# indrajeetadityaroy9/rabitq-ann-search

Hardware: AMD Instinct MI355X
Metric: qps (search_batch_device, layer-0 hot path end to end) + fastscan_dist_per_s (higher is better)
Workload: dtype u32 popcount / f32; 1 GPU; SIFT1M-class synthetic (int-valued, clustered; SURVEY 8d C2): 1000000x128 f32 (D=128), 4-bit RaBitQ FastScan + exact-L2 rerank, R=32, k=10, 10000 queries per GPU resident in HBM; n_index=1000000, dim=128, bits=4, k=10, nq_per_gpu=10000, index_builder=cphnsw_mi355x (this repo), batch_sets=2, parallelism=query-sharded x1, index replicated

## Files before the change

include/cphnsw_mi355x.h:

```cpp
#ifndef CPHNSW_MI355X_H
#define CPHNSW_MI355X_H

#include <stddef.h>
#include <stdint.h>

#ifdef __cplusplus
extern "C" {
#endif

typedef struct cph_index cph_index;

typedef enum {
    CPH_OK = 0,
    CPH_INVALID_ARGUMENT = 1,
    CPH_RUNTIME_ERROR = 2,
    CPH_OUT_OF_MEMORY = 3,
    CPH_NOT_IMPLEMENTED = 4
} cph_status;

const char* cph_last_error(void);

int cph_version(void);

int cph_create(uint64_t dim, uint64_t bits, int device, cph_index** out);
// ... 293 lines not shown
                                        int64_t* d_ids, float* d_dist, void* stream);
int cph_parts_search_batch_filters_device(cph_parts* m, const float* d_queries, uint64_t n, uint64_t k,
                                          const cph_parts_filter* const* filters, uint32_t n_filters, const int32_t* filter_of,
                                          int exact, int64_t* d_ids, float* d_dist, void* stream);
int cph_parts_search(cph_parts* m, const float* query, uint64_t k, int64_t* ids, float* dist, uint64_t* count);
int cph_parts_set_exact_threshold(cph_parts* m, uint64_t max_allowed);
int cph_parts_filter_create_rows(cph_parts* m, const uint32_t* words, uint64_t n_bits, cph_parts_filter** out);
int cph_parts_filter_destroy(cph_parts_filter* f);
int cph_parts_last_search_stats(cph_parts* m, uint64_t out[13]);
int cph_parts_last_query_expansions(cph_parts* m, uint32_t* out, uint64_t n);
int cph_parts_remove(cph_parts* m, const int64_t* ids, uint64_t cnt, uint64_t* newly);
int cph_parts_live_count(cph_parts* m, uint64_t* n);
int cph_parts_get_removed(cph_parts* m, uint32_t* words);
int cph_parts_compact(cph_parts* m, int64_t* old_to_new);
int cph_multi_set_labels(cph_multi* m, const int32_t* labels, uint64_t n, int space);
int cph_parts_set_labels(cph_parts* m, const int32_t* labels, uint64_t n);
int cph_parts_filters_from_labels(cph_parts* m, const int32_t* lo, const int32_t* hi, uint32_t cnt, cph_parts_filter** out);
int cph_parts_filter_count(const cph_parts_filter* f, uint64_t* count);
int cph_multi_set_column(cph_multi* m, uint32_t slot, const int32_t* values, uint64_t n, int space);
int cph_parts_set_column(cph_parts* m, uint32_t slot, const int32_t* values, uint64_t n);
int cph_parts_filters_from_column(cph_parts* m, uint32_t slot, const int32_t* lo, const int32_t* hi, uint32_t cnt, cph_parts_filter** out);
int cph_parts_filters_combine(int op, const cph_parts_filter* const* a, uint32_t m, const cph_parts_filter* const* b, uint32_t n_b,
                              cph_parts_filter** out);
int cph_parts_num_parts(cph_parts* m, uint32_t* n);
int cph_parts_part(cph_parts* m, uint32_t i, cph_index** out);
int cph_parts_bounds(cph_parts* m, uint64_t* out);
int cph_merge_rows_hook(int device, const int64_t* ids, const float* dist, uint32_t P, uint64_t n, uint64_t k, const int64_t* lo,
                        int64_t* out_ids, float* out_dist);

int cph_encode_query(cph_index* h, const float* query, uint8_t* lut, float* coeffs);

int cph_entry_point(cph_index* h, const float* query, uint32_t* entry);

int cph_fastscan_block(cph_index* h, const uint8_t* lut, const float* qparams,
                       uint32_t vertex, float dist_qp_sq, float worst, int nn_full,
                       uint32_t* sums, uint32_t* msb, float* est, float* lower,
                       float* lower_stage1);

int cph_exact_l2(cph_index* h, const float* query, const uint32_t* ids, uint64_t n,
                 float* out);

typedef struct cph_stream cph_stream;
int cph_fastscan_stream_create(int device, uint32_t D, uint32_t bits, uint64_t n_blocks,
                               uint64_t seed, cph_stream** out, uint64_t* block_bytes);
int cph_fastscan_stream_run(cph_stream* s, int reps, double* avg_ms, double* checksum);
int cph_fastscan_stream_export(cph_stream* s, uint64_t first, uint64_t count,
                               uint8_t* ref_blocks, uint8_t* lut, float* qparams,
                               float* dist_qp_sq);
int cph_fastscan_stream_eval(cph_stream* s, uint64_t first, uint64_t count, float* est,
                             float* lower);
int cph_fastscan_stream_destroy(cph_stream* s);

int cph_host_rewrite_index(const char* path_in, const char* path_out);
int cph_host_repack_block(uint32_t D, uint32_t bits, const uint8_t* ref_block, uint8_t* dev_block,
                          uint64_t* dev_bytes, uint8_t* ref_roundtrip);
int cph_host_relayout_block(uint32_t D, uint32_t bits, const uint8_t* dev_block, uint8_t* resident_block,
                            uint8_t* dev_roundtrip);
int cph_export_blocks(cph_index* h, uint64_t first, uint64_t count, int resident, uint8_t* out);
int cph_host_encode_query(uint64_t dim, const float* query, uint8_t* lut, float* coeffs, uint32_t* masks);
int cph_host_rows_filter(const uint32_t* words_in, const uint32_t* rows, uint64_t n, uint32_t* words_out);

int cph_host_live_filter(const uint32_t* words_f, const uint32_t* words_removed, uint64_t n, uint32_t* words_out,
                         uint64_t* count_out);

int cph_host_filter_ids(const uint32_t* words, uint64_t n_bits, uint32_t* out_ids, uint64_t* out_count);
int cph_host_exact_plan(uint64_t candidates, uint64_t n_queries, uint64_t k, int num_cus, uint64_t scratch_bytes, uint64_t* out);
// ... 60 lines not shown
```

rabitq-ann-search_amd/cphnsw_mi355x/_lib.py:

```python
import ctypes as C
import importlib.util
import os
import sys

from . import build as _build

OK, INVALID_ARGUMENT, RUNTIME_ERROR, OUT_OF_MEMORY, NOT_IMPLEMENTED = range(5)
IDS_INTERNAL, IDS_INPUT = 0, 1
METRIC_L2, METRIC_COSINE = 0, 1
METRIC_IP = 2

SYMBOLS = {
    "cph_last_error": (C.c_char_p, []),
    "cph_version": (C.c_int, []),
    "cph_create": (C.c_int, [C.c_uint64, C.c_uint64, C.c_int, C.POINTER(C.c_void_p)]),
    "cph_destroy": (C.c_int, [C.c_void_p]),
    "cph_load": (C.c_int, [C.c_void_p, C.c_char_p]),
    "cph_save": (C.c_int, [C.c_void_p, C.c_char_p]),
    "cph_save_native": (C.c_int, [C.c_void_p, C.c_char_p]),
    "cph_load_native": (C.c_int, [C.c_void_p, C.c_char_p]),
    "cph_size": (C.c_int, [C.c_void_p, C.POINTER(C.c_uint64)]),
    "cph_dim": (C.c_int, [C.c_void_p, C.POINTER(C.c_uint64)]),
    "cph_is_finalized": (C.c_int, [C.c_void_p, C.POINTER(C.c_int)]),
    "cph_build": (C.c_int, [C.c_void_p, C.c_void_p, C.c_uint64]),
# ... 201 lines not shown
    "cph_parts_size": (C.c_int, [C.c_void_p, C.POINTER(C.c_uint64)]),
    "cph_parts_is_finalized": (C.c_int, [C.c_void_p, C.POINTER(C.c_int)]),
    "cph_parts_save_native": (C.c_int, [C.c_void_p, C.c_char_p]),
    "cph_parts_load_native": (C.c_int, [C.c_void_p, C.c_char_p]),
    "cph_parts_search_batch": (C.c_int, [C.c_void_p, C.c_void_p, C.c_uint64, C.c_uint64, C.c_void_p, C.c_void_p]),
    "cph_parts_search_batch_filtered": (C.c_int, [C.c_void_p, C.c_void_p, C.c_uint64, C.c_uint64, C.c_void_p, C.c_void_p,
                                                  C.c_void_p]),
    "cph_parts_search_batch_exact": (C.c_int, [C.c_void_p, C.c_void_p, C.c_uint64, C.c_uint64, C.c_void_p, C.c_void_p,
                                               C.c_void_p]),
    "cph_parts_search_batch_filters": (C.c_int, [C.c_void_p, C.c_void_p, C.c_uint64, C.c_uint64, C.c_void_p, C.c_uint32,
                                                 C.c_void_p, C.c_int, C.c_void_p, C.c_void_p]),
    "cph_parts_search_batch_device": (C.c_int, [C.c_void_p, C.c_void_p, C.c_uint64, C.c_uint64, C.c_void_p, C.c_void_p,
                                                C.c_void_p]),
    "cph_parts_search_batch_device_filtered": (C.c_int, [C.c_void_p, C.c_void_p, C.c_uint64, C.c_uint64, C.c_void_p,
                                                         C.c_void_p, C.c_void_p, C.c_void_p]),
    "cph_parts_search_batch_exact_device": (C.c_int, [C.c_void_p, C.c_void_p, C.c_uint64, C.c_uint64, C.c_void_p,
                                                      C.c_void_p, C.c_void_p, C.c_void_p]),
    "cph_parts_search_batch_filters_device": (C.c_int, [C.c_void_p, C.c_void_p, C.c_uint64, C.c_uint64, C.c_void_p, C.c_uint32,
                                                        C.c_void_p, C.c_int, C.c_void_p, C.c_void_p, C.c_void_p]),
    "cph_parts_search": (C.c_int, [C.c_void_p, C.c_void_p, C.c_uint64, C.c_void_p, C.c_void_p, C.POINTER(C.c_uint64)]),
    "cph_parts_set_exact_threshold": (C.c_int, [C.c_void_p, C.c_uint64]),
    "cph_parts_filter_create_rows": (C.c_int, [C.c_void_p, C.c_void_p, C.c_uint64, C.POINTER(C.c_void_p)]),
    "cph_parts_filter_destroy": (C.c_int, [C.c_void_p]),
    "cph_parts_last_search_stats": (C.c_int, [C.c_void_p, C.POINTER(C.c_uint64)]),
    "cph_parts_last_query_expansions": (C.c_int, [C.c_void_p, C.c_void_p, C.c_uint64]),
    "cph_parts_num_parts": (C.c_int, [C.c_void_p, C.POINTER(C.c_uint32)]),
    "cph_parts_part": (C.c_int, [C.c_void_p, C.c_uint32, C.POINTER(C.c_void_p)]),
    "cph_parts_bounds": (C.c_int, [C.c_void_p, C.c_void_p]),
    "cph_merge_rows_hook": (C.c_int, [C.c_int, C.c_void_p, C.c_void_p, C.c_uint32, C.c_uint64, C.c_uint64, C.c_void_p,
                                      C.c_void_p, C.c_void_p]),
    "cph_host_part_bounds": (C.c_int, [C.c_uint64, C.c_uint32, C.c_void_p]),
    "cph_encode_query": (C.c_int, [C.c_void_p, C.c_void_p, C.c_void_p, C.c_void_p]),
    "cph_entry_point": (C.c_int, [C.c_void_p, C.c_void_p, C.POINTER(C.c_uint32)]),
    "cph_fastscan_block": (C.c_int, [C.c_void_p, C.c_void_p, C.c_void_p, C.c_uint32, C.c_float, C.c_float,
                                     C.c_int, C.c_void_p, C.c_void_p, C.c_void_p, C.c_void_p, C.c_void_p]),
    "cph_exact_l2": (C.c_int, [C.c_void_p, C.c_void_p, C.c_void_p, C.c_uint64, C.c_void_p]),
    "cph_host_rewrite_index": (C.c_int, [C.c_char_p, C.c_char_p]),
    "cph_host_repack_block": (C.c_int, [C.c_uint32, C.c_uint32, C.c_void_p, C.c_void_p, C.POINTER(C.c_uint64), C.c_void_p]),
    "cph_host_relayout_block": (C.c_int, [C.c_uint32, C.c_uint32, C.c_void_p, C.c_void_p, C.c_void_p]),
    "cph_export_blocks": (C.c_int, [C.c_void_p, C.c_uint64, C.c_uint64, C.c_int, C.c_void_p]),
    "cph_host_encode_query": (C.c_int, [C.c_uint64, C.c_void_p, C.c_void_p, C.c_void_p, C.c_void_p]),
    "cph_host_rows_filter": (C.c_int, [C.c_void_p, C.c_void_p, C.c_uint64, C.c_void_p]),
    "cph_fastscan_stream_create": (C.c_int, [C.c_int, C.c_uint32, C.c_uint32, C.c_uint64, C.c_uint64,
                                             C.POINTER(C.c_void_p), C.POINTER(C.c_uint64)]),
    "cph_fastscan_stream_run": (C.c_int, [C.c_void_p, C.c_int, C.POINTER(C.c_double), C.POINTER(C.c_double)]),
    "cph_fastscan_stream_export": (C.c_int, [C.c_void_p, C.c_uint64, C.c_uint64, C.c_void_p, C.c_void_p,
                                             C.c_void_p, C.POINTER(C.c_float)]),
    "cph_fastscan_stream_eval": (C.c_int, [C.c_void_p, C.c_uint64, C.c_uint64, C.c_void_p, C.c_void_p]),
    "cph_fastscan_stream_destroy": (C.c_int, [C.c_void_p]),
    "cph_set_metric": (C.c_int, [C.c_void_p, C.c_int]),
    "cph_get_metric": (C.c_int, [C.c_void_p, C.POINTER(C.c_int)]),
    "cph_multi_set_metric": (C.c_int, [C.c_void_p, C.c_int]),
    "cph_parts_set_metric": (C.c_int, [C.c_void_p, C.c_int]),
    "cph_metric_stats": (C.c_int, [C.c_void_p, C.POINTER(C.c_uint64)]),
    "cph_normalize_rows_hook": (C.c_int, [C.c_int, C.c_void_p, C.c_uint64, C.c_uint64, C.c_void_p, C.POINTER(C.c_uint64),
                                          C.POINTER(C.c_uint64)]),
    "cph_host_normalize_rows": (C.c_int, [C.c_void_p, C.c_uint64, C.c_uint64, C.c_void_p, C.POINTER(C.c_uint64),
                                          C.POINTER(C.c_uint64)]),
    "cph_set_metric_ip": (C.c_int, [C.c_void_p]),
    "cph_multi_set_metric_ip": (C.c_int, [C.c_void_p]),
    "cph_set_ip_bound": (C.c_int, [C.c_void_p, C.c_float]),
    "cph_get_ip_bound": (C.c_int, [C.c_void_p, C.POINTER(C.c_float)]),
    "cph_multi_set_ip_bound": (C.c_int, [C.c_void_p, C.c_float]),
    "cph_multi_get_ip_bound": (C.c_int, [C.c_void_p, C.POINTER(C.c_float)]),
    "cph_ip_augment_hook": (C.c_int, [C.c_int, C.c_void_p, C.c_uint64, C.c_uint64, C.c_int, C.c_float, C.c_void_p, C.c_void_p,
                                      C.POINTER(C.c_float), C.POINTER(C.c_uint64)]),
# ... 83 lines not shown
```

rabitq-ann-search_amd/cphnsw_mi355x/build.py:

```python
import os
import shutil
import subprocess

PKG_DIR = os.path.dirname(os.path.abspath(__file__))
CSRC = os.path.join(os.path.dirname(PKG_DIR), "csrc")
LIB_PATH = os.path.join(PKG_DIR, "libcphnsw_mi355x.so")
SOURCES = ["cphnsw_mi355x.hip"]
HEADERS = ["cph_core.h", "builder.h", "builder_host.h", "host_parallel.h", "search_coalescer.h", "multi_device.h", "partitioned.h", "device_merge.h", "builder_pipeline.h", "device_knn.h", "device_knn_sym.h", "device_build.h", "device_buf.h", "native_file.h", "device_encode.h", "device_fastscan.h", "device_search.h", "device_search_expansion.inc", "device_stream.h", "device_heap_test.h", "device_relayout.h", "device_rows.h", "device_tombstone.h", "device_labels.h", "device_filter_ops.h", "device_exact.h", "device_range.h", "device_tail.h", "host_tail.h", "device_group.h", "host_group.h", "device_diverse.h", "host_diverse.h", "device_maxsim.h", "host_maxsim.h", "device_maxsim_rescore.h", "host_maxsim_rescore.h", "device_fused.h", "host_fused.h", "device_normalize.h", "host_normalize.h", "device_ip.h", "host_ip.h", "device_rescore.h", "host_rescore.h", "host_index.h"]
FLAGS = ["-O3", "-std=c++17", "--offload-arch=gfx950", "-fPIC", "-shared", "-ffp-contract=off",
         "-Wall", "-Wno-unused-function"]


def _hipcc():
    for c in (os.environ.get("HIPCC"), shutil.which("hipcc"), "/opt/rocm/bin/hipcc"):
        if c and os.path.exists(c):
            return c
    raise RuntimeError("hipcc not found (need ROCm to build the gfx950 library)")


def needs_build():
    if not os.path.exists(LIB_PATH):
        return True
    t = os.path.getmtime(LIB_PATH)
    deps = [os.path.join(CSRC, f) for f in SOURCES + HEADERS]
    deps.append(os.path.join(os.path.dirname(os.path.dirname(PKG_DIR)), "include", "cphnsw_mi355x.h"))
    return any(os.path.getmtime(d) > t for d in deps if os.path.exists(d))


def build_library(force=False, verbose=False):
    if not force and not needs_build():
        return LIB_PATH
    cmd = [_hipcc()] + FLAGS + [os.path.join(CSRC, s) for s in SOURCES] + ["-o", LIB_PATH, "-lpthread"]
    if verbose:
        print(" ".join(cmd))
    subprocess.check_call(cmd)
    return LIB_PATH


if __name__ == "__main__":
    print(build_library(force=True, verbose=True))
```

rabitq-ann-search_amd/csrc/cphnsw_mi355x.hip:

```cpp
#include <hip/hip_runtime.h>

#include <algorithm>
#include <atomic>
#include <cfloat>
#include <chrono>
#include <condition_variable>
#include <deque>
#include <functional>
#include <memory>
#include <mutex>
#include <new>
#include <shared_mutex>
#include <string>
#include <thread>
#include <vector>

#include "../../include/cphnsw_mi355x.h"
#include "cph_core.h"
#include "device_buf.h"
#include "device_encode.h"
#include "device_fastscan.h"
#include "device_search.h"
#include "device_stream.h"
#include "device_heap_test.h"
#include "device_relayout.h"
#include "device_rows.h"
#include "device_tombstone.h"
#include "device_labels.h"
#include "device_filter_ops.h"
#include "device_exact.h"
#include "device_range.h"
#include "device_tail.h"
#include "device_diverse.h"
#include "device_group.h"
#include "device_maxsim.h"
#include "device_maxsim_rescore.h"
#include "device_fused.h"
#include "device_rescore.h"
#include "device_normalize.h"
#include "device_ip.h"
#include "host_index.h"
#include "host_parallel.h"
#include "search_coalescer.h"
#include "multi_device.h"
#include "partitioned.h"
#include "device_merge.h"
#include "native_file.h"
#include "builder_pipeline.h"

using namespace cph;

namespace {

thread_local std::string g_err;

int fail(int code, const std::string& msg) {
    g_err = msg;
    return code;
}

struct InvalidArg : std::invalid_argument {
    using std::invalid_argument::invalid_argument;
};
struct NotImplemented : std::runtime_error {
    using std::runtime_error::runtime_error;
};

template <class F>
int guarded(F&& f) {
    try {
        f();
        return CPH_OK;
    } catch (const std::invalid_argument& e) {
// ... 157 lines not shown
    float ip_bound = 0.0f, ip_m2 = 0.0f;
    std::vector<float> pending;
    uint64_t pending_n = 0;
    HostIndex host;
    DevLayout L{};
    SearchConsts sc{};
    uint32_t flags = 0;
    int num_cus = 256;
    bool waves_from_env = false;
    uint32_t waves_per_cu = 4 * CPH_SEARCH_WAVES_PER_SIMD;
    DevBuf<uint8_t> d_blocks;
    DevBuf<float> d_raw, d_norm;
    DevBuf<uint32_t> d_rows;
    bool has_rows = false;
    bool ids_input = false;
    DevBuf<int32_t> d_labels, d_label_bounds;
    DevBuf<unsigned long long> d_label_counts;
    bool has_labels = false;
    std::unique_ptr<KeyRows> label_rows;
    DevBuf<int32_t> d_columns[kMaxColumns];
    bool has_column[kMaxColumns] = {};
    size_t exact_scratch_bytes = (size_t)1 << 30;
    uint64_t exact_threshold = 0;
    DevBuf<uint32_t> d_removed;
    DevBuf<unsigned long long> d_rm_count;
    uint64_t rm_epoch = 0;
    std::shared_ptr<cph_filter> live;
    std::atomic<bool> tombstones{false};
    uint64_t tail = 0;
    std::vector<float> tail_vecs;
    std::atomic<bool> has_tail{false};
    DevBuf<float> d_signs;
    DevBuf<uint32_t> d_upper;
    DevBuf<uint32_t> d_row_of;
    DevBuf<uint32_t> d_nbr_info;
    UpperLayerDev layers[kMaxUpperLayers];
    int32_t dev_max_level = 0;
    float norm_factor = 0.0f, inv_sqrt_d = 0.0f;
    NativeMapping native_map;
    const uint8_t* own_view = nullptr;
    std::vector<uint8_t> own_store;
    BatchSet sets[kMaxBatchSets + kLeaderSlots];
    int n_sets = 2;
    int last_set = kMaxBatchSets - 1;
    int last_search = -1;
    bool last_range = false;
    uint64_t range_exact = 0;
    std::vector<std::unique_ptr<RangeScratch>> range_scratch;
    GroupScratch group_scratch[kMaxBatchSets];
    int last_group = kMaxBatchSets - 1;
    struct PassTimer {
        hipEvent_t ev0 = nullptr, ev1 = nullptr;
        bool on = false, timed = false;
    } pass_timer[kPassKinds];
    uint64_t index_epoch = 0;
    hipStream_t own_stream = nullptr;
    bool order_queries = true;
    uint32_t want_slots = 0;
    uint64_t want_cap = 0;
    uint64_t auto_cap = 0;
    bool pf_off = false;
    bool pf_dense = false;
    std::mutex mu;
    SearchCoalescer coal;
    struct LeaderSlot {
        hipStream_t stream = nullptr;
        uint8_t* pin = nullptr;
        uint8_t* pin_dev = nullptr;
// ... 234 lines not shown
    if (n != 0) {
        DevBuf<uint32_t> d_flag(1);
        HIP_CHECK(hipMemset(d_flag.p, 0, 4));
        hipLaunchKernelGGL(scan_counts_kernel, dim3((uint32_t)((n + 255) / 256)), dim3(256), 0, nullptr, h->d_blocks.p, (uint64_t)n,
                           h->L.stride, h->L.count_off, d_flag.p);
        HIP_CHECK(hipGetLastError());
        uint32_t f = 0;
        HIP_CHECK(hipMemcpy(&f, d_flag.p, 4, hipMemcpyDeviceToHost));
        h->flags |= f & 2u;
    }
    h->d_signs.alloc(3 * hi.D);
    HIP_CHECK(hipMemcpy(h->d_signs.p, hi.rot.signs.data(), 3 * hi.D * 4, hipMemcpyHostToDevice));
    const float d = static_cast<float>(hi.D);
    h->norm_factor = 1.0f / (d * std::sqrt(d));
    h->inv_sqrt_d = 1.0f / std::sqrt(d);
    const int nl = std::min<int>({(int)hi.upper.size(), (int)hi.max_level, kMaxUpperLayers});
    h->dev_max_level = hi.max_level > 0 ? nl : 0;
    std::vector<uint32_t> flat;
    std::vector<size_t> off_nodes(nl), off_offs(nl), off_nbrs(nl);
    for (int l = 0; l < nl; ++l) {
        const auto& layer = hi.upper[l];
        off_nodes[l] = flat.size();
        for (const auto& e : layer) flat.push_back(e.node);
        off_offs[l] = flat.size();
        uint32_t acc = 0;
        for (const auto& e : layer) { flat.push_back(acc); acc += (uint32_t)e.nbrs.size(); }
        flat.push_back(acc);
        off_nbrs[l] = flat.size();
        for (const auto& e : layer) flat.insert(flat.end(), e.nbrs.begin(), e.nbrs.end());
    }
    h->d_upper.alloc(flat.size() + 1);
    if (!flat.empty())
        HIP_CHECK(hipMemcpy(h->d_upper.p, flat.data(), flat.size() * 4, hipMemcpyHostToDevice));
    for (int l = 0; l < kMaxUpperLayers; ++l) h->layers[l] = UpperLayerDev{nullptr, nullptr, nullptr, nullptr, nullptr, 0};
    int mapped = 0;
    size_t mapped_edges = 0;
    for (int l = 0; l < nl; ++l) {
        if (hi.upper[l].size() <= 16) continue;
        ++mapped;
        for (const auto& e : hi.upper[l]) mapped_edges += e.nbrs.size();
    }
    h->d_row_of.alloc((size_t)mapped * n + 1);
    h->d_nbr_info.alloc(mapped_edges + 1);
    std::vector<uint32_t> row_of, nbr_info;
    size_t info_off = 0;
    for (int l = 0, m = 0; l < nl; ++l) {
        const uint32_t* dmap = nullptr;
        const uint32_t* dinfo = nullptr;
        if (hi.upper[l].size() > 16) {
            row_of.assign(n, kInvalidNode);
            uint64_t first = 0;
            bool fits = true;
            for (size_t r = 0; r < hi.upper[l].size(); ++r) {
                const uint64_t deg = hi.upper[l][r].nbrs.size();
                if (first >= (1u << 26) || deg > 62) { fits = false; break; }
                row_of[hi.upper[l][r].node] = (uint32_t)first | ((uint32_t)deg << 26);
                first += deg;
            }
            if (!fits) { h->layers[l] = UpperLayerDev{h->d_upper.p + off_nodes[l], h->d_upper.p + off_offs[l], h->d_upper.p + off_nbrs[l], nullptr, nullptr, (uint32_t)hi.upper[l].size()}; ++m; continue; }
            HIP_CHECK(hipMemcpy(h->d_row_of.p + (size_t)m * n, row_of.data(), n * 4, hipMemcpyHostToDevice));
            dmap = h->d_row_of.p + (size_t)m * n;
            ++m;
            nbr_info.clear();
            for (const auto& e : hi.upper[l])
                for (const uint32_t nb : e.nbrs) nbr_info.push_back(nb < n ? row_of[nb] : kInvalidNode);
            if (info_off + nbr_info.size() > mapped_edges) throw std::runtime_error("upper layers: edge count changed during upload");
            if (!nbr_info.empty())
                HIP_CHECK(hipMemcpy(h->d_nbr_info.p + info_off, nbr_info.data(), nbr_info.size() * 4, hipMemcpyHostToDevice));
            dinfo = h->d_nbr_info.p + info_off;
            info_off += nbr_info.size();
        }
        h->layers[l] = UpperLayerDev{h->d_upper.p + off_nodes[l], h->d_upper.p + off_offs[l],
                                     h->d_upper.p + off_nbrs[l], dmap, dinfo, (uint32_t)hi.upper[l].size()};
    }
    for (auto& s : h->sets) release_scratch(s);
    reset_adaptation(h);
}

void materialize_search_data(cph_index* h) {
    HostIndex& hi = h->host;
    if (!hi.search_data.empty() || hi.n == 0) return;
    h->use_device();
    quiesce(h);
    const size_t n = hi.n, stride = h->L.stride, own_stride = hi.RL.nb_off;
    hi.search_data.assign(n * hi.RL.vertex_bytes, 0);
    const size_t chunk = std::max<size_t>(1, std::min<size_t>(n, (512u << 20) / stride));
    std::vector<uint8_t> stage(chunk * stride);
    for (size_t base = 0; base < n; base += chunk) {
        const size_t c = std::min(chunk, n - base);
        download_blocks(h->d_blocks.p + base * stride, c, h->L, stage.data());
        parallel_for(c, 256, [&](size_t lo, size_t hi_) {
            for (size_t v = lo; v < hi_; ++v) {
                uint8_t* dst = &hi.search_data[(base + v) * hi.RL.vertex_bytes];
                if (h->own_view) std::memcpy(dst, h->own_view + (base + v) * own_stride, own_stride);
                repack_dev_to_ref(&stage[v * stride], h->L, hi.RL, dst + hi.RL.nb_off);
            }
        });
    }
}

void init_set(BatchSet& s) {
    if (s.ev0) return;
    HIP_CHECK(hipEventCreate(&s.ev0));
    HIP_CHECK(hipEventCreate(&s.ev1));
    HIP_CHECK(hipEventCreateWithFlags(&s.ev_done, hipEventDisableTiming));
    HIP_CHECK(hipHostMalloc(reinterpret_cast<void**>(&s.pin_stats), kStatWords * 8, hipHostMallocDefault));
    std::memset(s.pin_stats, 0, kStatWords * 8);
// ... 2650 lines not shown
        const uint32_t D = h->D, PW = h->L.PW;
        std::vector<uint32_t> masks(PW * 4);
        QueryHeader hd;
        HIP_CHECK(hipMemcpy(masks.data(), s.d_qmasks.p, PW * 16, hipMemcpyDeviceToHost));
        HIP_CHECK(hipMemcpy(&hd, s.d_qhdr.p, sizeof(hd), hipMemcpyDeviceToHost));
        std::vector<uint8_t> qu(D);
        for (uint32_t d = 0; d < D; ++d) {
            uint8_t u = 0;
            for (int j = 0; j < 4; ++j) u |= (uint8_t)(((masks[(d / 32) * 4 + j] >> (d % 32)) & 1u) << j);
            qu[d] = u;
        }
        qu_to_lut(qu.data(), D, lut);
        coeffs[0] = hd.A; coeffs[1] = hd.B; coeffs[2] = hd.C;
    });
}

int cph_entry_point(cph_index* h, const float* query, uint32_t* entry) {
    return guarded([&] {
        std::lock_guard<std::mutex> lk(h->mu);
        require_finalized(h);
        h->use_device();
        hipStream_t st = own_stream(h);
        BatchSet& s = next_set(h, st);
        stage_queries(h, s, upload_queries(h, s, query, 1, st, true), 1, st);
        HIP_CHECK(hipEventRecord(s.ev_done, st));
        s.used = true;
        HIP_CHECK(hipStreamSynchronize(st));
        QueryHeader hd;
        HIP_CHECK(hipMemcpy(&hd, s.d_qhdr.p, sizeof(hd), hipMemcpyDeviceToHost));
        *entry = hd.entry;
    });
}

int cph_fastscan_block(cph_index* h, const uint8_t* lut, const float* qparams, uint32_t vertex,
                       float dist_qp_sq, float worst, int nn_full, uint32_t* sums, uint32_t* msb,
                       float* est, float* lower, float* lower_stage1) {
    return guarded([&] {
        std::lock_guard<std::mutex> lk(h->mu);
        require_finalized(h);
        if (vertex >= h->host.n) throw InvalidArg("vertex out of range");
        h->use_device();
        const uint32_t D = h->D, PW = h->L.PW;
        std::vector<uint8_t> qu(D);
        lut_to_qu(lut, D, qu.data());
        std::vector<uint32_t> masks(PW * 4);
        qu_to_masks(qu.data(), D, masks.data());
        DevBuf<uint4> d_mask;
        DevBuf<uint32_t> d_u;
        DevBuf<float> d_f;
        d_mask.alloc(PW);
        d_u.alloc(64);
        d_f.alloc(96);
        HIP_CHECK(hipMemcpy(d_mask.p, masks.data(), PW * 16, hipMemcpyHostToDevice));
        BlockHookArgs a{};
        a.blk = h->d_blocks.p + (size_t)vertex * h->L.stride;
        a.L = h->L;
        a.qmask = d_mask.p;
        a.qp = QP{qparams[0], qparams[1], qparams[2], qparams[3], qparams[4], qparams[5], qparams[6]};
        a.dqp = dist_qp_sq;
        a.worst = worst;
        a.nn_full = nn_full;
        a.sums = d_u.p; a.msb = d_u.p + 32;
        a.est = d_f.p; a.lower = d_f.p + 32; a.lower1 = d_f.p + 64;
        CPH_LAUNCH(block_hook_kernel, h->bits, D, dim3(1), dim3(64), (size_t)PW * 16, nullptr, a);
        HIP_CHECK(hipDeviceSynchronize());
        uint32_t hu[64];
// ... 373 lines not shown
    HIP_CHECK(hipDeviceSynchronize());
    begin_device_swap(dst);
    dst->host = host_scalars(src->host);
    dst->host.removed = src->host.removed;
    dst->host.n_removed = src->host.n_removed;
    drop_host_state(dst);
    dst->L = src->L;
    dst->sc = src->sc;
    dst->flags = src->flags;
    dst->dev_max_level = src->dev_max_level;
    dst->norm_factor = src->norm_factor;
    dst->inv_sqrt_d = src->inv_sqrt_d;
    dst->ip_m2 = src->ip_m2;
    hipStream_t st = own_stream(dst);
    auto copy = [&](auto& d, const auto& s) {
        d.alloc(s.n);
        if (s.n) HIP_CHECK(hipMemcpyPeerAsync(d.p, dst->device, s.p, src->device, s.n * sizeof(*s.p), st));
    };
    copy(dst->d_blocks, src->d_blocks);
    copy(dst->d_raw, src->d_raw);
    copy(dst->d_norm, src->d_norm);
    if (src->has_rows) copy(dst->d_rows, src->d_rows);
    else dst->d_rows.release();
    dst->has_rows = src->has_rows;
    dst->ids_input = dst->ids_input && dst->has_rows;
    for (int slot = kLabelSlot; slot < (int)kMaxColumns; ++slot) {
        const ColumnRef from = column_of(src, slot), to = column_of(dst, slot);
        if (from.has) copy(to.dev, from.dev);
        else to.dev.release();
        to.has = from.has;
    }
    copy(dst->d_signs, src->d_signs);
    copy(dst->d_upper, src->d_upper);
    copy(dst->d_row_of, src->d_row_of);
    copy(dst->d_nbr_info, src->d_nbr_info);
    HIP_CHECK(hipStreamSynchronize(st));
    sync_removed(dst);
    auto rebase = [](const uint32_t* p, const DevBuf<uint32_t>& from, const DevBuf<uint32_t>& to) -> const uint32_t* {
        return p ? to.p + (p - from.p) : nullptr;
    };
    for (int l = 0; l < kMaxUpperLayers; ++l) {
        const UpperLayerDev& s = src->layers[l];
        dst->layers[l] = UpperLayerDev{rebase(s.nodes, src->d_upper, dst->d_upper), rebase(s.offsets, src->d_upper, dst->d_upper),
                                       rebase(s.nbrs, src->d_upper, dst->d_upper), rebase(s.row_of, src->d_row_of, dst->d_row_of),
                                       rebase(s.nbr_info, src->d_nbr_info, dst->d_nbr_info), s.n_nodes};
    }
    reset_adaptation(dst);
    dst->finalized = true;
}

template <class F>
void multi_lifecycle(cph_multi* m, F&& first) {
    std::unique_lock<std::shared_mutex> lk(m->life);
    cph_index* r0 = m->reps[0];
    bool first_done = false;
    try {
        first(r0);
        first_done = true;
        for (size_t i = 1; i < m->reps.size(); ++i) replicate(r0, m->reps[i]);
    } catch (...) {
        if (first_done || !r0->finalized)
            for (cph_index* h : m->reps) {
                std::lock_guard<std::mutex> g(h->mu);
                h->finalized = false;
            }
        throw;
    }
}

size_t shard_index(const std::vector<Shard>& plan, const Shard& s) {
    for (size_t i = 0; i < plan.size(); ++i)
        if (plan[i].replica == s.replica && plan[i].lo == s.lo && plan[i].hi == s.hi) return i;
    throw std::runtime_error("shard not in the plan");
}

template <class Call>
void run_shards(cph_multi* m, const std::vector<Shard>& plan, Call&& call) {
    std::string err;
// ... 3278 lines not shown
```

rabitq-ann-search_amd/csrc/device_encode.h:

```cpp
#pragma once
#include <hip/hip_runtime.h>

#include <cstddef>

#include "cph_core.h"
#include "device_fastscan.h"

namespace cph {

struct UpperLayerDev {
    const uint32_t* nodes;
    const uint32_t* offsets;
    const uint32_t* nbrs;
    const uint32_t* row_of;
    const uint32_t* nbr_info;
    uint32_t n_nodes;
};

constexpr int kMaxUpperLayers = 24;

struct EncodeArgs {
    const float* queries_raw;
    uint32_t nq, dim, D, PW;
    const float* signs;
    float norm_factor, inv_sqrt_d;
    const float* raw;
    uint64_t n;
    uint32_t entry;
    int32_t max_level;
    UpperLayerDev layers[kMaxUpperLayers];
    float* queries_padded;
    uint4* qmasks;
    QueryHeader* qhdr;
    float* entry_dist;
};

__device__ __forceinline__ void wave_fht(float* x, uint32_t D, int lane) {
    for (uint32_t h = 1; h < D; h <<= 1) {
        for (uint32_t b = lane; b < D / 2; b += 64) {
            const uint32_t i = (b / h) * 2 * h + (b % h);
            const float lo = x[i], hi = x[i + h];
            x[i] = lo + hi;
            x[i + h] = (h < 8) ? (hi - lo) : (lo - hi);
        }
        __syncthreads();
    }
}

// ... 4 lines not shown
    for (int j = 0; j < N; ++j) r[j] = *reinterpret_cast<const float4*>(v + 8 * j);
#pragma unroll
    for (int j = 0; j < QR; ++j) q[j] = *reinterpret_cast<const float4*>(q_lds + 8 * j);
    __builtin_amdgcn_sched_barrier(0);
#pragma unroll
    for (int j = 0; j < N; ++j) {
        const float4 qq = q[j % QR];
        const float d0 = qq.x - r[j].x, d1 = qq.y - r[j].y, d2 = qq.z - r[j].z, d3 = qq.w - r[j].w;
        c[0] = __fmaf_rn(d0, d0, c[0]);
        c[1] = __fmaf_rn(d1, d1, c[1]);
        c[2] = __fmaf_rn(d2, d2, c[2]);
        c[3] = __fmaf_rn(d3, d3, c[3]);
        if (j + QR < N) q[j % QR] = *reinterpret_cast<const float4*>(q_lds + 8 * (j + QR));
        __builtin_amdgcn_sched_barrier(0);
    }
}
__device__ __forceinline__ float pair_reduce(const float (&c)[4]) {
    const float s0 = c[0] + dpp_mov<0xB1>(c[0]), s1 = c[1] + dpp_mov<0xB1>(c[1]);
    const float s2 = c[2] + dpp_mov<0xB1>(c[2]), s3 = c[3] + dpp_mov<0xB1>(c[3]);
    return (s0 + s1) + (s2 + s3);
}

__device__ __forceinline__ void min_step(float& cand, uint32_t& pos, float od, uint32_t op) {
    if (od < cand || (od == cand && op < pos)) { cand = od; pos = op; }
}
template <int CTRL>
__device__ __forceinline__ void min_step_dpp(float& cand, uint32_t& pos) {
    min_step(cand, pos, dpp_mov<CTRL>(cand), (uint32_t)__builtin_amdgcn_update_dpp(0, (int)pos, CTRL, 0xF, 0xF, true));
}
__device__ __forceinline__ float uniform_f32(float v) {
    return __builtin_bit_cast(float, __builtin_amdgcn_readfirstlane(__builtin_bit_cast(int, v)));
}
__device__ __forceinline__ uint32_t uniform_u32(uint32_t v) { return (uint32_t)__builtin_amdgcn_readfirstlane((int)v); }
__device__ __forceinline__ void min_rows(float& cand, uint32_t& pos) {
    float bc = uniform_f32(cand);
    uint32_t bp = uniform_u32(pos);
#pragma unroll
    for (int r = 16; r < 64; r += 16)
        min_step(bc, bp, __builtin_bit_cast(float, __builtin_amdgcn_readlane(__builtin_bit_cast(int, cand), r)),
                 (uint32_t)__builtin_amdgcn_readlane((int)pos, r));
    cand = bc;
    pos = bp;
}
__device__ __forceinline__ int fresh_lane(int lane) {
    asm volatile("" : "+v"(lane));
    return lane;
}

__device__ __forceinline__ UpperLayerDev load_layer(int idx) {
    static_assert(sizeof(UpperLayerDev) == 48 && offsetof(UpperLayerDev, n_nodes) == 40, "six qwords per descriptor");
    using kbyte = const __attribute__((address_space(4))) unsigned char;
    using kqword = const __attribute__((address_space(4))) uint64_t;
    kbyte* seg = (kbyte*)__builtin_amdgcn_kernarg_segment_ptr();
    kqword* w = reinterpret_cast<kqword*>(seg + offsetof(EncodeArgs, layers) + (size_t)idx * sizeof(UpperLayerDev));
    UpperLayerDev L;
    L.nodes = reinterpret_cast<const uint32_t*>(w[0]);
    L.offsets = reinterpret_cast<const uint32_t*>(w[1]);
    L.nbrs = reinterpret_cast<const uint32_t*>(w[2]);
    L.row_of = reinterpret_cast<const uint32_t*>(w[3]);
    L.nbr_info = reinterpret_cast<const uint32_t*>(w[4]);
    L.n_nodes = (uint32_t)w[5];
    return L;
}

__host__ __device__ inline size_t encode_lds_bytes(uint32_t D) { return (size_t)D * 8; }

__global__ __launch_bounds__(64) void encode_kernel(EncodeArgs a) {
    extern __shared__ __align__(16) unsigned char smem[];
    float* qv = reinterpret_cast<float*>(smem);
    float* x = qv + a.D;
    const uint32_t D = a.D;
    for (uint32_t qi = blockIdx.x; qi < a.nq; qi += gridDim.x) {
        const int lane = fresh_lane(threadIdx.x);
        for (uint32_t d = lane; d < D; d += 64) {
            float v = d < a.dim ? a.queries_raw[(size_t)qi * a.dim + d] : 0.0f;
            qv[d] = v;
            x[d] = v;
            a.queries_padded[(size_t)qi * D + d] = v;
        }
        __syncthreads();
        for (int l = 0; l < 3; ++l) {
            for (uint32_t d = lane; d < D; d += 64) x[d] = x[d] * a.signs[l * D + d];
            __syncthreads();
            wave_fht(x, D, lane);
        }
        for (uint32_t d = lane; d < D; d += 64) x[d] = x[d] * a.norm_factor;
        __syncthreads();
        float vmin = x[lane < (int)D ? lane : 0], vmx = vmin;
        uint32_t imin = lane < (int)D ? lane : 0, imax = imin;
        for (uint32_t d = lane + 64; d < D; d += 64) {
            const float v = x[d];
            if (v < vmin) { vmin = v; imin = d; }
            if (v > vmx) { vmx = v; imax = d; }
// ... 11 lines not shown
        float delta = (vh - vl) / 15.0f;
        if (delta < kEpsTiny) delta = kEpsTiny;
        const float inv_delta = 1.0f / delta;
        uint32_t usum = 0;
        for (uint32_t base = 0; base < D; base += 64) {
            const uint32_t d = base + lane;
            int u = 0;
            if (d < D) {
                u = (int)__fmaf_rn(x[d] - vl, inv_delta, 0.5f);
                u = u < 0 ? 0 : (u > 15 ? 15 : u);
            }
            usum += (uint32_t)u;
            const unsigned long long b0 = __ballot(u & 1), b1 = __ballot(u & 2), b2 = __ballot(u & 4),
                                     b3 = __ballot(u & 8);
            if (lane == 0) {
                const uint32_t w = base / 32;
                a.qmasks[(size_t)qi * a.PW + w] =
                    make_uint4((uint32_t)b0, (uint32_t)b1, (uint32_t)b2, (uint32_t)b3);
                if (w + 1 < a.PW)
                    a.qmasks[(size_t)qi * a.PW + w + 1] = make_uint4(
                        (uint32_t)(b0 >> 32), (uint32_t)(b1 >> 32), (uint32_t)(b2 >> 32), (uint32_t)(b3 >> 32));
            }
        }
        for (int o = 1; o < 64; o <<= 1) usum += __shfl_xor(usum, o);
        const float sum_qu = (float)usum;
        const float df = (float)D;
        QueryHeader hd;
        hd.A = uniform_f32((2.0f * delta) * a.inv_sqrt_d);
        hd.B = uniform_f32((2.0f * vl) * a.inv_sqrt_d);
        hd.C = uniform_f32(-__fmaf_rn(df, vl, delta * sum_qu) * a.inv_sqrt_d);

        uint32_t ep = a.entry;
        float ep_dist = 0.0f;
        if (a.max_level > 0 && ep < a.n) {
            const bool paired = (D % 128u) == 0;
            for (int level = a.max_level; level >= 1; --level) {
                const UpperLayerDev Ly = load_layer(level - 1);
                float best = (level == a.max_level)
                                 ? uniform_f32(group_l2sq8(qv, a.raw + (size_t)ep * D, D, fresh_lane(lane) & 7))
                                 : ep_dist;
                uint32_t best_id = ep;
                if (Ly.row_of) {
                    uint32_t info = Ly.row_of[best_id];
                    while (info != kInvalidNode) {
                        const uint32_t beg = info & 0x03FFFFFFu, cnt = info >> 26;
                        float cand = 3.402823466e+38f;
                        uint32_t cand_pos = 0xFFFFFFFFu;
                        uint32_t mine = best_id, mine_info = kInvalidNode, src;
                        if (paired && cnt <= 32) {
                            const int pl = fresh_lane(lane);
                            const uint32_t p = (uint32_t)pl >> 1;
                            const int half = pl & 1;
                            const bool have = p < cnt;
                            float c[4] = {0.0f, 0.0f, 0.0f, 0.0f};
                            if (have) {
                                mine = Ly.nbrs[beg + p];
                                mine_info = Ly.nbr_info[beg + p];
                                const float* v = a.raw + (size_t)mine * D + 4 * half;
                                for (uint32_t base = 0; base < D; base += 64) pair_l2_part<8, 3>(qv + base + 4 * half, v + base, c);
                            }
                            const float d = pair_reduce(c);
                            if (have && d < cand) { cand = d; cand_pos = p; }
                            min_step_dpp<0x4E>(cand, cand_pos);
                            min_step_dpp<0x124>(cand, cand_pos);
                            min_step_dpp<0x128>(cand, cand_pos);
                            min_rows(cand, cand_pos);
                            src = cand_pos * 2;
                        } else {
                            const int sl = fresh_lane(lane);
                            if ((uint32_t)sl < cnt) {
                                mine = Ly.nbrs[beg + sl];
                                mine_info = Ly.nbr_info[beg + sl];
                            }
                            for (uint32_t base = 0; base < cnt; base += 8) {
                                const uint32_t pos = base + (sl >> 3);
                                const bool have = pos < cnt;
                                const uint32_t nb = (uint32_t)__shfl((int)mine, (int)(have ? pos : 0));
                                const float d = group_l2sq8(qv, a.raw + (size_t)(have ? nb : best_id) * D, D, sl & 7);
                                if (have && (d < cand || (d == cand && pos < cand_pos))) { cand = d; cand_pos = pos; }
                            }
                            for (int o = 8; o < 64; o <<= 1) {
                                const float od = __shfl_xor(cand, o);
                                const uint32_t op = __shfl_xor(cand_pos, o);
                                if (od < cand || (od == cand && op < cand_pos)) { cand = od; cand_pos = op; }
                            }
                            cand = uniform_f32(cand);
                            src = cand_pos = uniform_u32(cand_pos);
                        }
                        if (cand_pos == 0xFFFFFFFFu || !(cand < best)) break;
                        best = cand;
                        best_id = (uint32_t)__builtin_amdgcn_readlane((int)mine, (int)src);
                        info = (uint32_t)__builtin_amdgcn_readlane((int)mine_info, (int)src);
                    }
                } else {
                    bool improved = true;
                    while (improved) {
                        improved = false;
                        float cand = 3.402823466e+38f;
                        uint32_t cand_id = kInvalidNode;
                        uint32_t cand_pos = 0xFFFFFFFFu;
                        uint32_t lo = 0, hi = Ly.n_nodes;
                        while (lo < hi) {
                            const uint32_t mid = (lo + hi) >> 1;
                            if (Ly.nodes[mid] < best_id) lo = mid + 1; else hi = mid;
                        }
                        if (lo >= Ly.n_nodes || Ly.nodes[lo] != best_id) break;
                        const uint32_t beg = Ly.offsets[lo], end = Ly.offsets[lo + 1];
                        const int sl = fresh_lane(lane);
                        for (uint32_t base = beg; base < end; base += 8) {
                            const uint32_t pos = base + (sl >> 3);
                            const bool have = pos < end;
                            const uint32_t nb = have ? Ly.nbrs[pos] : best_id;
                            const float d = group_l2sq8(qv, a.raw + (size_t)nb * D, D, sl & 7);
                            if (have && (d < cand || (d == cand && pos < cand_pos))) {
                                cand = d; cand_id = nb; cand_pos = pos;
                            }
                        }
                        for (int o = 8; o < 64; o <<= 1) {
                            const float od = __shfl_xor(cand, o);
                            const uint32_t oi = __shfl_xor(cand_id, o);
                            const uint32_t op = __shfl_xor(cand_pos, o);
                            if (od < cand || (od == cand && op < cand_pos)) { cand = od; cand_id = oi; cand_pos = op; }
                        }
                        cand = uniform_f32(cand);
                        cand_id = uniform_u32(cand_id);
                        if (cand_id != kInvalidNode && cand < best) {
// ... 59 lines not shown
```

Measured before the change: 6.800 million queries/s.

## Replace per-layer row_of map with packed descent rows carrying next-layer info

Upper-layer greedy descent now uses a single packed uint2 row array per layer. Each row has a header word giving the same node's row in the layer below, followed by (neighbor, neighbor-row-info) pairs. This removes the dense n-sized row_of lookup at every level transition and the separate nbrs/nbr_info loads, replacing them with one scalar load of the header and one interleaved 8-byte load per edge. The entry node's info is precomputed per layer, and the old dense per-layer maps of n entries are dropped, saving memory. The layout requires strict validation (sorted nodes, degree at most 62, nested layers) and otherwise falls back to the binary-search path.

```diff
diff --git a/include/cphnsw_mi355x.h b/include/cphnsw_mi355x.h
--- a/include/cphnsw_mi355x.h
+++ b/include/cphnsw_mi355x.h
@@ -349,6 +349,9 @@
 
 int cph_entry_point(cph_index* h, const float* query, uint32_t* entry);
 
+int cph_host_descent_rows(uint32_t n_layers, const uint32_t* n_nodes, const uint32_t* nodes, const uint32_t* offsets, const uint32_t* nbrs,
+                          uint64_t n, uint32_t entry, uint32_t* rows_out, uint64_t* first_out, uint32_t* entry_info_out, int* usable_out);
+
 int cph_fastscan_block(cph_index* h, const uint8_t* lut, const float* qparams,
                        uint32_t vertex, float dist_qp_sq, float worst, int nn_full,
                        uint32_t* sums, uint32_t* msb, float* est, float* lower,
diff --git a/rabitq-ann-search_amd/cphnsw_mi355x/_lib.py b/rabitq-ann-search_amd/cphnsw_mi355x/_lib.py
--- a/rabitq-ann-search_amd/cphnsw_mi355x/_lib.py
+++ b/rabitq-ann-search_amd/cphnsw_mi355x/_lib.py
@@ -257,6 +257,8 @@
     "cph_host_part_bounds": (C.c_int, [C.c_uint64, C.c_uint32, C.c_void_p]),
     "cph_encode_query": (C.c_int, [C.c_void_p, C.c_void_p, C.c_void_p, C.c_void_p]),
     "cph_entry_point": (C.c_int, [C.c_void_p, C.c_void_p, C.POINTER(C.c_uint32)]),
+    "cph_host_descent_rows": (C.c_int, [C.c_uint32, C.c_void_p, C.c_void_p, C.c_void_p, C.c_void_p, C.c_uint64, C.c_uint32, C.c_void_p, C.c_void_p,
+                                        C.c_void_p, C.POINTER(C.c_int)]),
     "cph_fastscan_block": (C.c_int, [C.c_void_p, C.c_void_p, C.c_void_p, C.c_uint32, C.c_float, C.c_float,
                                      C.c_int, C.c_void_p, C.c_void_p, C.c_void_p, C.c_void_p, C.c_void_p]),
     "cph_exact_l2": (C.c_int, [C.c_void_p, C.c_void_p, C.c_void_p, C.c_uint64, C.c_void_p]),
diff --git a/rabitq-ann-search_amd/cphnsw_mi355x/build.py b/rabitq-ann-search_amd/cphnsw_mi355x/build.py
--- a/rabitq-ann-search_amd/cphnsw_mi355x/build.py
+++ b/rabitq-ann-search_amd/cphnsw_mi355x/build.py
@@ -6,7 +6,7 @@
 CSRC = os.path.join(os.path.dirname(PKG_DIR), "csrc")
 LIB_PATH = os.path.join(PKG_DIR, "libcphnsw_mi355x.so")
 SOURCES = ["cphnsw_mi355x.hip"]
-HEADERS = ["cph_core.h", "builder.h", "builder_host.h", "host_parallel.h", "search_coalescer.h", "multi_device.h", "partitioned.h", "device_merge.h", "builder_pipeline.h", "device_knn.h", "device_knn_sym.h", "device_build.h", "device_buf.h", "native_file.h", "device_encode.h", "device_fastscan.h", "device_search.h", "device_search_expansion.inc", "device_stream.h", "device_heap_test.h", "device_relayout.h", "device_rows.h", "device_tombstone.h", "device_labels.h", "device_filter_ops.h", "device_exact.h", "device_range.h", "device_tail.h", "host_tail.h", "device_group.h", "host_group.h", "device_diverse.h", "host_diverse.h", "device_maxsim.h", "host_maxsim.h", "device_maxsim_rescore.h", "host_maxsim_rescore.h", "device_fused.h", "host_fused.h", "device_normalize.h", "host_normalize.h", "device_ip.h", "host_ip.h", "device_rescore.h", "host_rescore.h", "host_index.h"]
+HEADERS = ["cph_core.h", "host_descent.h", "builder.h", "builder_host.h", "host_parallel.h", "search_coalescer.h", "multi_device.h", "partitioned.h", "device_merge.h", "builder_pipeline.h", "device_knn.h", "device_knn_sym.h", "device_build.h", "device_buf.h", "native_file.h", "device_encode.h", "device_fastscan.h", "device_search.h", "device_search_expansion.inc", "device_stream.h", "device_heap_test.h", "device_relayout.h", "device_rows.h", "device_tombstone.h", "device_labels.h", "device_filter_ops.h", "device_exact.h", "device_range.h", "device_tail.h", "host_tail.h", "device_group.h", "host_group.h", "device_diverse.h", "host_diverse.h", "device_maxsim.h", "host_maxsim.h", "device_maxsim_rescore.h", "host_maxsim_rescore.h", "device_fused.h", "host_fused.h", "device_normalize.h", "host_normalize.h", "device_ip.h", "host_ip.h", "device_rescore.h", "host_rescore.h", "host_index.h"]
 FLAGS = ["-O3", "-std=c++17", "--offload-arch=gfx950", "-fPIC", "-shared", "-ffp-contract=off",
          "-Wall", "-Wno-unused-function"]
 
diff --git a/rabitq-ann-search_amd/csrc/cphnsw_mi355x.hip b/rabitq-ann-search_amd/csrc/cphnsw_mi355x.hip
--- a/rabitq-ann-search_amd/csrc/cphnsw_mi355x.hip
+++ b/rabitq-ann-search_amd/csrc/cphnsw_mi355x.hip
@@ -39,6 +39,7 @@
 #include "device_rescore.h"
 #include "device_normalize.h"
 #include "device_ip.h"
+#include "host_descent.h"
 #include "host_index.h"
 #include "host_parallel.h"
 #include "search_coalescer.h"
@@ -262,8 +263,7 @@
     std::atomic<bool> has_tail{false};
     DevBuf<float> d_signs;
     DevBuf<uint32_t> d_upper;
-    DevBuf<uint32_t> d_row_of;
-    DevBuf<uint32_t> d_nbr_info;
+    DevBuf<uint2> d_descent_rows;
     UpperLayerDev layers[kMaxUpperLayers];
     int32_t dev_max_level = 0;
     float norm_factor = 0.0f, inv_sqrt_d = 0.0f;
@@ -564,47 +564,23 @@
     h->d_upper.alloc(flat.size() + 1);
     if (!flat.empty())
         HIP_CHECK(hipMemcpy(h->d_upper.p, flat.data(), flat.size() * 4, hipMemcpyHostToDevice));
-    for (int l = 0; l < kMaxUpperLayers; ++l) h->layers[l] = UpperLayerDev{nullptr, nullptr, nullptr, nullptr, nullptr, 0};
-    int mapped = 0;
-    size_t mapped_edges = 0;
-    for (int l = 0; l < nl; ++l) {
-        if (hi.upper[l].size() <= 16) continue;
-        ++mapped;
-        for (const auto& e : hi.upper[l]) mapped_edges += e.nbrs.size();
-    }
-    h->d_row_of.alloc((size_t)mapped * n + 1);
-    h->d_nbr_info.alloc(mapped_edges + 1);
-    std::vector<uint32_t> row_of, nbr_info;
-    size_t info_off = 0;
-    for (int l = 0, m = 0; l < nl; ++l) {
-        const uint32_t* dmap = nullptr;
-        const uint32_t* dinfo = nullptr;
-        if (hi.upper[l].size() > 16) {
-            row_of.assign(n, kInvalidNode);
-            uint64_t first = 0;
-            bool fits = true;
-            for (size_t r = 0; r < hi.upper[l].size(); ++r) {
-                const uint64_t deg = hi.upper[l][r].nbrs.size();
-                if (first >= (1u << 26) || deg > 62) { fits = false; break; }
-                row_of[hi.upper[l][r].node] = (uint32_t)first | ((uint32_t)deg << 26);
-                first += deg;
-            }
-            if (!fits) { h->layers[l] = UpperLayerDev{h->d_upper.p + off_nodes[l], h->d_upper.p + off_offs[l], h->d_upper.p + off_nbrs[l], nullptr, nullptr, (uint32_t)hi.upper[l].size()}; ++m; continue; }
-            HIP_CHECK(hipMemcpy(h->d_row_of.p + (size_t)m * n, row_of.data(), n * 4, hipMemcpyHostToDevice));
-            dmap = h->d_row_of.p + (size_t)m * n;
-            ++m;
-            nbr_info.clear();
-            for (const auto& e : hi.upper[l])
-                for (const uint32_t nb : e.nbrs) nbr_info.push_back(nb < n ? row_of[nb] : kInvalidNode);
-            if (info_off + nbr_info.size() > mapped_edges) throw std::runtime_error("upper layers: edge count changed during upload");
-            if (!nbr_info.empty())
-                HIP_CHECK(hipMemcpy(h->d_nbr_info.p + info_off, nbr_info.data(), nbr_info.size() * 4, hipMemcpyHostToDevice));
-            dinfo = h->d_nbr_info.p + info_off;
-            info_off += nbr_info.size();
-        }
-        h->layers[l] = UpperLayerDev{h->d_upper.p + off_nodes[l], h->d_upper.p + off_offs[l],
-                                     h->d_upper.p + off_nbrs[l], dmap, dinfo, (uint32_t)hi.upper[l].size()};
-    }
+    for (int l = 0; l < kMaxUpperLayers; ++l) h->layers[l] = UpperLayerDev{};
+    std::vector<LayerCsr> csr(nl);
+    for (int l = 0; l < nl; ++l)
+        csr[l] = LayerCsr{flat.data() + off_nodes[l], flat.data() + off_offs[l], flat.data() + off_nbrs[l], (uint32_t)hi.upper[l].size()};
+    const char* env_rows = getenv("CPH_DESCENT_ROWS");
+    DescentRows rows;
+    if (!(env_rows && atoi(env_rows) == 0) && h->dev_max_level > 0) rows = descent_rows(csr, n, hi.entry);
+    const bool use_rows = rows.usable && !rows.words.empty();
+    h->d_descent_rows.release();
+    if (use_rows) {
+        h->d_descent_rows.alloc(rows.words.size() / 2);
+        HIP_CHECK(hipMemcpy(h->d_descent_rows.p, rows.words.data(), rows.words.size() * 4, hipMemcpyHostToDevice));
+    }
+    for (int l = 0; l < nl; ++l)
+        h->layers[l] = UpperLayerDev{h->d_upper.p + off_nodes[l], h->d_upper.p + off_offs[l], h->d_upper.p + off_nbrs[l],
+                                     use_rows ? h->d_descent_rows.p + rows.first[l] : nullptr, use_rows ? rows.entry_info[l] : kInvalidNode,
+                                     0, csr[l].n_nodes};
     for (auto& s : h->sets) release_scratch(s);
     reset_adaptation(h);
 }
@@ -3321,6 +3297,29 @@
     });
 }
 
+int cph_host_descent_rows(uint32_t n_layers, const uint32_t* n_nodes, const uint32_t* nodes, const uint32_t* offsets, const uint32_t* nbrs,
+                          uint64_t n, uint32_t entry, uint32_t* rows_out, uint64_t* first_out, uint32_t* entry_info_out, int* usable_out) {
+    return guarded([&] {
+        if (!first_out || !usable_out || (n_layers && (!n_nodes || !nodes || !offsets || !nbrs || !rows_out || !entry_info_out)))
+            throw InvalidArg("null argument");
+        if (n_layers > (uint32_t)kMaxUpperLayers) throw InvalidArg("too many layers");
+        if (n > 0xFFFFFFFFull) throw InvalidArg("bad n");
+        std::vector<LayerCsr> csr(n_layers);
+        for (uint32_t l = 0; l < n_layers; ++l) {
+            if (offsets[0] != 0) throw InvalidArg("a layer's offsets start at 0");
+            csr[l] = LayerCsr{nodes, offsets, nbrs, n_nodes[l]};
+            nodes += n_nodes[l];
+            nbrs += offsets[n_nodes[l]];
+            offsets += (size_t)n_nodes[l] + 1;
+        }
+        const DescentRows rows = descent_rows(csr, n, entry);
+        std::copy(rows.words.begin(), rows.words.end(), rows_out);
+        std::copy(rows.first.begin(), rows.first.end(), first_out);
+        std::copy(rows.entry_info.begin(), rows.entry_info.end(), entry_info_out);
+        *usable_out = rows.usable ? 1 : 0;
+    });
+}
+
 int cph_fastscan_block(cph_index* h, const uint8_t* lut, const float* qparams, uint32_t vertex,
                        float dist_qp_sq, float worst, int nn_full, uint32_t* sums, uint32_t* msb,
                        float* est, float* lower, float* lower_stage1) {
@@ -3760,18 +3759,17 @@
     }
     copy(dst->d_signs, src->d_signs);
     copy(dst->d_upper, src->d_upper);
-    copy(dst->d_row_of, src->d_row_of);
-    copy(dst->d_nbr_info, src->d_nbr_info);
+    copy(dst->d_descent_rows, src->d_descent_rows);
     HIP_CHECK(hipStreamSynchronize(st));
     sync_removed(dst);
-    auto rebase = [](const uint32_t* p, const DevBuf<uint32_t>& from, const DevBuf<uint32_t>& to) -> const uint32_t* {
+    auto rebase = [](const auto* p, const auto& from, const auto& to) -> decltype(p) {
         return p ? to.p + (p - from.p) : nullptr;
     };
     for (int l = 0; l < kMaxUpperLayers; ++l) {
         const UpperLayerDev& s = src->layers[l];
         dst->layers[l] = UpperLayerDev{rebase(s.nodes, src->d_upper, dst->d_upper), rebase(s.offsets, src->d_upper, dst->d_upper),
-                                       rebase(s.nbrs, src->d_upper, dst->d_upper), rebase(s.row_of, src->d_row_of, dst->d_row_of),
-                                       rebase(s.nbr_info, src->d_nbr_info, dst->d_nbr_info), s.n_nodes};
+                                       rebase(s.nbrs, src->d_upper, dst->d_upper), rebase(s.rows, src->d_descent_rows, dst->d_descent_rows),
+                                       s.entry_info, 0, s.n_nodes};
     }
     reset_adaptation(dst);
     dst->finalized = true;
diff --git a/rabitq-ann-search_amd/csrc/device_encode.h b/rabitq-ann-search_amd/csrc/device_encode.h
--- a/rabitq-ann-search_amd/csrc/device_encode.h
+++ b/rabitq-ann-search_amd/csrc/device_encode.h
@@ -12,8 +12,9 @@
     const uint32_t* nodes;
     const uint32_t* offsets;
     const uint32_t* nbrs;
-    const uint32_t* row_of;
-    const uint32_t* nbr_info;
+    const uint2* rows;
+    uint32_t entry_info;
+    uint32_t unused;
     uint32_t n_nodes;
 };
 
@@ -84,6 +85,10 @@
     return __builtin_bit_cast(float, __builtin_amdgcn_readfirstlane(__builtin_bit_cast(int, v)));
 }
 __device__ __forceinline__ uint32_t uniform_u32(uint32_t v) { return (uint32_t)__builtin_amdgcn_readfirstlane((int)v); }
+__device__ __forceinline__ uint32_t uniform_load(const uint32_t* p) {
+    using kword = const __attribute__((address_space(4))) uint32_t;
+    return *reinterpret_cast<kword*>(reinterpret_cast<uintptr_t>(p));
+}
 __device__ __forceinline__ void min_rows(float& cand, uint32_t& pos) {
     float bc = uniform_f32(cand);
     uint32_t bp = uniform_u32(pos);
@@ -109,8 +114,8 @@
     L.nodes = reinterpret_cast<const uint32_t*>(w[0]);
     L.offsets = reinterpret_cast<const uint32_t*>(w[1]);
     L.nbrs = reinterpret_cast<const uint32_t*>(w[2]);
-    L.row_of = reinterpret_cast<const uint32_t*>(w[3]);
-    L.nbr_info = reinterpret_cast<const uint32_t*>(w[4]);
+    L.rows = reinterpret_cast<const uint2*>(w[3]);
+    L.entry_info = (uint32_t)w[4];
     L.n_nodes = (uint32_t)w[5];
     return L;
 }
@@ -188,6 +193,7 @@
 
         uint32_t ep = a.entry;
         float ep_dist = 0.0f;
+        uint32_t info = kInvalidNode;
         if (a.max_level > 0 && ep < a.n) {
             const bool paired = (D % 128u) == 0;
             for (int level = a.max_level; level >= 1; --level) {
@@ -196,10 +202,14 @@
                                  ? uniform_f32(group_l2sq8(qv, a.raw + (size_t)ep * D, D, fresh_lane(lane) & 7))
                                  : ep_dist;
                 uint32_t best_id = ep;
-                if (Ly.row_of) {
-                    uint32_t info = Ly.row_of[best_id];
+                if (Ly.rows) {
+                    if (level == a.max_level) info = Ly.entry_info;
+                    uint32_t below = kInvalidNode;
                     while (info != kInvalidNode) {
-                        const uint32_t beg = info & 0x03FFFFFFu, cnt = info >> 26;
+                        const uint32_t row = uniform_u32(info);
+                        const uint32_t beg = row & 0x03FFFFFFu, cnt = row >> 26;
+                        below = uniform_load(&Ly.rows[beg].x);
+                        const uint2* edges = Ly.rows + beg + 1;
                         float cand = 3.402823466e+38f;
                         uint32_t cand_pos = 0xFFFFFFFFu;
                         uint32_t mine = best_id, mine_info = kInvalidNode, src;
@@ -210,8 +220,9 @@
                             const bool have = p < cnt;
                             float c[4] = {0.0f, 0.0f, 0.0f, 0.0f};
                             if (have) {
-                                mine = Ly.nbrs[beg + p];
-                                mine_info = Ly.nbr_info[beg + p];
+                                const uint2 e = edges[p];
+                                mine = e.x;
+                                mine_info = e.y;
                                 const float* v = a.raw + (size_t)mine * D + 4 * half;
                                 for (uint32_t base = 0; base < D; base += 64) pair_l2_part<8, 3>(qv + base + 4 * half, v + base, c);
                             }
@@ -225,8 +236,9 @@
                         } else {
                             const int sl = fresh_lane(lane);
                             if ((uint32_t)sl < cnt) {
-                                mine = Ly.nbrs[beg + sl];
-                                mine_info = Ly.nbr_info[beg + sl];
+                                const uint2 e = edges[sl];
+                                mine = e.x;
+                                mine_info = e.y;
                             }
                             for (uint32_t base = 0; base < cnt; base += 8) {
                                 const uint32_t pos = base + (sl >> 3);
@@ -243,11 +255,13 @@
                             cand = uniform_f32(cand);
                             src = cand_pos = uniform_u32(cand_pos);
                         }
+                        asm volatile("" : "+s"(below));
                         if (cand_pos == 0xFFFFFFFFu || !(cand < best)) break;
                         best = cand;
                         best_id = (uint32_t)__builtin_amdgcn_readlane((int)mine, (int)src);
                         info = (uint32_t)__builtin_amdgcn_readlane((int)mine_info, (int)src);
                     }
+                    info = info == kInvalidNode ? kInvalidNode : below;
                 } else {
                     bool improved = true;
                     while (improved) {
diff --git a/rabitq-ann-search_amd/csrc/host_descent.h b/rabitq-ann-search_amd/csrc/host_descent.h
--- /dev/null
+++ b/rabitq-ann-search_amd/csrc/host_descent.h
@@ -0,0 +1,82 @@
+#pragma once
+#include <algorithm>
+#include <cstddef>
+#include <cstdint>
+#include <vector>
+
+#include "cph_core.h"
+
+namespace cph {
+
+struct LayerCsr {
+    const uint32_t* nodes;
+    const uint32_t* offsets;
+    const uint32_t* nbrs;
+    uint32_t n_nodes;
+};
+
+constexpr uint32_t kRowOffsetBits = 26;
+constexpr uint32_t kRowMaxDegree = 62;
+
+struct DescentRows {
+    std::vector<uint32_t> words;
+    std::vector<uint64_t> first;
+    std::vector<uint32_t> entry_info;
+    bool usable = true;
+};
+
+inline uint32_t descent_info(const LayerCsr& L, uint64_t v) {
+    const uint32_t* end = L.nodes + L.n_nodes;
+    const uint32_t* it = std::lower_bound(L.nodes, end, v, [](uint32_t a, uint64_t b) { return a < b; });
+    if (it == end || *it != v) return kInvalidNode;
+    const size_t r = (size_t)(it - L.nodes);
+    const uint32_t beg = L.offsets[r], deg = L.offsets[r + 1] - L.offsets[r];
+    return ((beg + (uint32_t)r) & ((1u << kRowOffsetBits) - 1)) | (deg << kRowOffsetBits);
+}
+
+inline bool descent_rows_usable(const std::vector<LayerCsr>& layers, uint64_t n, uint32_t entry) {
+    for (size_t l = 0; l < layers.size(); ++l) {
+        const LayerCsr& L = layers[l];
+        if (entry >= n || descent_info(L, entry) == kInvalidNode) return false;
+        const uint64_t edges = L.offsets[L.n_nodes];
+        if ((uint64_t)L.n_nodes + edges > ((uint64_t)1 << kRowOffsetBits)) return false;
+        for (uint32_t r = 0; r < L.n_nodes; ++r) {
+            if (L.nodes[r] >= n || (r != 0 && L.nodes[r] <= L.nodes[r - 1])) return false;
+            if (L.offsets[r + 1] < L.offsets[r] || L.offsets[r + 1] - L.offsets[r] > kRowMaxDegree) return false;
+        }
+    }
+    for (size_t l = 1; l < layers.size(); ++l)
+        for (uint32_t r = 0; r < layers[l].n_nodes; ++r)
+            if (descent_info(layers[l - 1], layers[l].nodes[r]) == kInvalidNode) return false;
+    return true;
+}
+
+inline DescentRows descent_rows(const std::vector<LayerCsr>& layers, uint64_t n, uint32_t entry) {
+    DescentRows out;
+    out.usable = descent_rows_usable(layers, n, entry);
+    out.first.assign(layers.size() + 1, 0);
+    out.entry_info.assign(layers.size(), kInvalidNode);
+    if (!out.usable) return out;
+    for (size_t l = 0; l < layers.size(); ++l) out.first[l + 1] = out.first[l] + layers[l].n_nodes + layers[l].offsets[layers[l].n_nodes];
+    out.words.resize(2 * out.first.back());
+    uint32_t* w = out.words.data();
+    std::vector<uint32_t> cur, below;
+    for (size_t l = 0; l < layers.size(); ++l) {
+        const LayerCsr& L = layers[l];
+        cur.assign(n, kInvalidNode);
+        for (uint32_t r = 0; r < L.n_nodes; ++r) cur[L.nodes[r]] = (L.offsets[r] + r) | ((L.offsets[r + 1] - L.offsets[r]) << kRowOffsetBits);
+        out.entry_info[l] = cur[entry];
+        for (uint32_t r = 0; r < L.n_nodes; ++r) {
+            *w++ = l == 0 ? kInvalidNode : below[L.nodes[r]];
+            *w++ = 0;
+            for (uint32_t e = L.offsets[r]; e < L.offsets[r + 1]; ++e) {
+                *w++ = L.nbrs[e];
+                *w++ = L.nbrs[e] < n ? cur[L.nbrs[e]] : kInvalidNode;
+            }
+        }
+        below.swap(cur);
+    }
+    return out;
+}
+
+}
```

Result: no change. 6.789 million queries/s (-0.2%).
